# crabml/crabml

Measured on NVIDIA H100. Metric: decode_tokens_per_s, higher is better.
Workload: dtype int8

## Files before the change

### crabml_b200/csrc/mega.cu

```cuda
#define MK_SYNC() __syncthreads()
#include "mega_phases.cuh"

struct MkNextNorm { const float* norm_w; int norm_n; };

template <bool SMP>
__global__ void __launch_bounds__(MK_THREADS, MK_CTAS_PER_SM) mega_kernel(const MkPhase* __restrict__ phases, int n_phases, const uint8_t* dyn,
                                                                         unsigned* bar, const uint16_t* exp_lut, unsigned long long* prof, bool test_stall, int wtop_off,
                                                                         unsigned* err_host) {
    extern __shared__ __align__(16) uint8_t smem[];
    __shared__ float s_red[MK_WARPS];
    __shared__ MkPhase s_phs[2];
    __shared__ MkNextNorm s_next;
    __shared__ int s_abort;
    __shared__ __align__(8) unsigned long long s_abar[AT_NBUF];
    unsigned apar = 0u;
    const unsigned abar0 = (unsigned)__cvta_generic_to_shared(&s_abar[0]);
    if (threadIdx.x == 0) { for (int i = 0; i < AT_NBUF; i++) mbar_init(abar0 + 8u * i, 1u); s_abort = 0; }
    asm volatile("fence.mbarrier_init.release.cluster;" ::: "memory");
    asm volatile("fence.proxy.async.shared::cta;" ::: "memory");
    __syncthreads();
    const CommDev nocomm = {};
    KSeg S0, S1;
    uint8_t* work = smem;
    float* s_w = (float*)(smem + wtop_off);
    int wstaged = -1;
    int xstaged = -1;
    unsigned gen = 0;
    if (threadIdx.x == MK_BAR_THREAD) gen = ld_acquire_u32(&bar[32]);
    {
        const int* src = (const int*)phases;
        int* dst = (int*)&s_phs[0];
        for (int i = threadIdx.x; i < (int)(sizeof(MkPhase) / 4); i += MK_THREADS) dst[i] = src[i];
    }
    const int n_loop = SMP ? n_phases - 1 : n_phases;
    for (int p = 0; p < n_loop; p++) {
        const bool stamp = prof && blockIdx.x == 0 && threadIdx.x == 0;
        if (stamp) { prof[p * MK_PROF_SLOTS] = globaltimer_ns(); prof[p * MK_PROF_SLOTS + 1] = 0; prof[p * MK_PROF_SLOTS + 4] = 0; prof[p * MK_PROF_SLOTS + 5] = 0; }
        __syncthreads();
        const MkPhase& s_ph = s_phs[p & 1];
        static_assert(sizeof(MkPhase) / 4 <= MK_THREADS, "descriptor does not fit one word per thread");
        const int nx = s_ph.next_matvec;
        const bool look = nx > p && nx < n_phases;
        int desc_w = 0, next_w = 0;
        if (p + 1 < n_phases && threadIdx.x < sizeof(MkPhase) / 4) desc_w = ((const int*)(phases + p + 1))[threadIdx.x];
        if (look && threadIdx.x < 3) {
            const MkPhase* ph = phases + nx;
            next_w = threadIdx.x < 2 ? ((const int*)&ph->norm_w)[threadIdx.x] : ph->x && ph->norm_w && ph->norm_ahead ? ph->n : 0;
        }
        switch (s_ph.type) {
        case MK_NORMQ: phase_normq(s_ph, s_red); break;
        case MK_MATVEC: {
            unsigned long long* st1 = stamp ? prof + p * MK_PROF_SLOTS + 1 : nullptr;
            switch (s_ph.wtype) {
            case CC_Q2_K: phase_matvec_generic<TQ2_K>(s_ph, work, s_w, wstaged == p, xstaged == p, exp_lut, st1, S0, S1); break;
            case CC_Q3_K: phase_matvec_generic<TQ3_K>(s_ph, work, s_w, wstaged == p, xstaged == p, exp_lut, st1, S0, S1); break;
            case CC_Q4_K: phase_matvec_generic<TQ45_K<false>>(s_ph, work, s_w, wstaged == p, xstaged == p, exp_lut, st1, S0, S1); break;
            case CC_Q5_K: phase_matvec_generic<TQ45_K<true>>(s_ph, work, s_w, wstaged == p, xstaged == p, exp_lut, st1, S0, S1); break;
            case CC_Q6_K: phase_matvec_generic<TQ6_K>(s_ph, work, s_w, wstaged == p, xstaged == p, exp_lut, st1, S0, S1); break;
            default: phase_matvec_generic<TQ8_K>(s_ph, work, s_w, wstaged == p, xstaged == p, exp_lut, st1, S0, S1); break;
            }
            break;
        }
        case MK_ATTN:
            if (s_ph.at.kv_f16) phase_attn<true>(s_ph, (float*)work, s_red, dyn, exp_lut, abar0, apar, AT_CH); else phase_attn<false>(s_ph, (float*)work, s_red, dyn, exp_lut, abar0, apar, AT_CH);
            break;
        case MK_ROWS: phase_rows(s_ph, dyn); break;
        case MK_ARGMAX: phase_argmax(s_ph, dyn, s_red); break;
        }
        if (stamp) prof[p * MK_PROF_SLOTS + 2] = globaltimer_ns();
        if (p + 1 < n_phases && threadIdx.x < sizeof(MkPhase) / 4) ((int*)&s_phs[(p + 1) & 1])[threadIdx.x] = desc_w;
        if (look && threadIdx.x < 3) ((int*)&s_next)[threadIdx.x] = next_w;
        const bool more = p + 1 < n_phases;
        if (test_stall && p == 2 && blockIdx.x == gridDim.x - 1) { if (threadIdx.x == 0) s_abort = 1; break; }
        if (more) grid_barrier_arrive(bar, gridDim.x, gen);
        if (look && s_next.norm_n > 0) {
            const unsigned sw = (unsigned)__cvta_generic_to_shared(s_w);
            const float* nw = s_next.norm_w;
            for (int i = threadIdx.x; i < (s_next.norm_n >> 2); i += MK_THREADS)
                asm volatile("cp.async.cg.shared.global [%0], [%1], 16;" ::"r"(sw + i * 16), "l"(nw + i * 4) : "memory");
            asm volatile("cp.async.commit_group;" ::: "memory");
            wstaged = nx;
        }
        if (stamp) prof[p * MK_PROF_SLOTS + 3] = globaltimer_ns();
        if (more) {
            grid_barrier_wait(bar, gridDim.x, gen, nocomm, 0u, &s_abort, err_host);
            gen++;
            if (s_abort) break;
            const MkPhase& nph = s_phs[(p + 1) & 1];
            if (nph.type == MK_MATVEC && nph.x) {
                const unsigned sx = (unsigned)__cvta_generic_to_shared(work + mk_generic_sx_offset(nph.mv.k));
                const float* xg = nph.x;
                for (int i = threadIdx.x; i < (nph.mv.k >> 2); i += MK_THREADS)
                    asm volatile("cp.async.cg.shared.global [%0], [%1], 16;" ::"r"(sx + i * 16), "l"(xg + i * 4) : "memory");
                asm volatile("cp.async.commit_group;" ::: "memory");
                xstaged = p + 1;
            }
        }
    }
    asm volatile("cp.async.wait_all;" ::: "memory");
    if constexpr (SMP) {
        __syncthreads();
        if (!s_abort) phase_sample(s_phs[(n_phases - 1) & 1], dyn, work, exp_lut);
    }
    if (prof && blockIdx.x == 0 && threadIdx.x == 0) prof[n_phases * MK_PROF_SLOTS] = globaltimer_ns();
}

size_t cc_mega_smem_for_phase(const MkPhase& ph) {
    if (ph.type == MK_MATVEC) return (size_t)(((TKBase::smem_bytes(ph.mv.k) + 15) & ~15) + 256) + (size_t)ph.mv.k * 4;
    if (ph.type == MK_ATTN) return (size_t)(3 * ph.at.hd + ((ph.at.max_len + 8 + 3) & ~3) + AT_NBUF * AT_CH * ph.at.hd) * 4 + 64;
    if (ph.type == MK_SAMPLE) return SMP_SMEM_BYTES;
    return 1024;
}

extern "C" CC_API int cc_test_mega_barrier_floor(cc_device* dev, int n, float* us_per_phase) {
    if (!dev || n < 2 || !us_per_phase) return CC_ERR_ARG;
    std::vector<MkPhase> tab((size_t)n);
    for (auto& p : tab) { memset(&p, 0, sizeof(p)); p.type = 99; p.next_matvec = -1; }
// ... 49 lines not shown
```

### crabml_b200/csrc/mega_phases.cuh

```cuda
#pragma once
#include <stdlib.h>
#include <string.h>

#include "common.cuh"
#include "dequant.cuh"
#include "quantize_dev.cuh"
#include "vecdot.cuh"
#include "sample_dev.cuh"

#ifndef MK_SYNC
#error "define MK_SYNC() before including mega_phases.cuh"
#endif

#define MK_THREADS 512
#define MK_WARPS 16
#define MK_CTAS_PER_SM 1
#define MK_SEG 4
#define MK_XSTAGE_ROWS 512

__device__ __forceinline__ unsigned ld_acquire_u32(const unsigned* p) {
    unsigned v;
    asm volatile("ld.acquire.gpu.global.u32 %0, [%1];" : "=r"(v) : "l"(p) : "memory");
    return v;
}
// ... 203 lines not shown
    auto emit = [&](int i, float v) {
        int mat;
        const int r = locate(i, mat);
        if (pair) {
            if ((i & 1) == 0) { first = v; return; }
            flush_pending();
            if (lane == 0) { pend_a = first; pend_b = v; pend_row = r; pend_lut = exp_lut[f2h_bits(-first)]; }
        } else if (A.epilogue == 1) {
            flush_pending();
            if (lane == 0) { pend_a = v; pend_row = r; pend_res = ldcg_f(A.residual + r); }
        } else if (lane == 0) {
            float* o = mat == 0 ? M.out[0] : mat == 1 ? M.out[1] : M.out[2];
            o[r] = v;
        }
    };
    if constexpr (T::kSegmented) {
        const int NSEG = ((k >> 8) + 15) >> 4;
        const int U = n_vrows * NSEG;
#if MK_GENERIC_NOINLINE
        KSeg S0, S1;
#endif
        int x0[4] = {0, 0, 0, 0}, x1[4] = {0, 0, 0, 0};
        int l_i = 0, l_seg = 0;
        auto load = [&](KSeg& S, int (&x)[4], bool valid) {
            if (valid) { int mat; const int r = locate(l_i, mat); T::seg_load(S, x, planes(mat), r, k, l_seg, lane); }
            if (++l_seg == NSEG) { l_seg = 0; l_i++; }
        };
        load(S0, x0, U > 0);
        load(S1, x1, U > 1);
        float acc = 0.0f;
        int c_i = 0, c_seg = 0;
        auto finish = [&]() { if (++c_seg < NSEG) return; c_seg = 0; const float v = warp_sum(acc); acc = 0.0f; emit(c_i++, v); };
        for (int u = 0; u < U; u += 2) {
            acc = T::seg_dot(S0, x0, k, c_seg, smem, lane, acc);
            finish();
            load(S0, x0, u + 2 < U);
            if (u + 1 >= U) break;
            acc = T::seg_dot(S1, x1, k, c_seg, smem, lane, acc);
            finish();
            load(S1, x1, u + 3 < U);
        }
    } else {
        for (int i = 0; i < n_vrows; i++) {
            int mat;
            const int r = locate(i, mat);
            emit(i, warp_sum(T::row_dot(planes(mat), r, k, smem, lane)));
        }
    }
    flush_pending();
}

#define AT_CH 64
#define AT_NBUF 3
template <bool KV_F16>
static __device__ void phase_attn(const MkPhase& ph, float* sm, float* s_red, const uint8_t* dyn, const uint16_t* exp_lut, unsigned abar0, unsigned& apar, const int at_ch) {
    const AttnArgs& a = ph.at;
    const int n_heads = a.n_heads, n_kv = a.n_kv, hd = a.hd, rope_dim = a.rope_dim;
    const int64_t seq_stride = a.seq_stride;
    const int64_t* dynv = (const int64_t*)(dyn + ph.dyn_off);
    const float* rope_tab = (const float*)(dyn + ph.rope_off);
    const int kv_len = (int)dynv[1], L = kv_len + 1;
    const int lane = threadIdx.x & 31, warp = threadIdx.x >> 5;
    float* s_q = sm; float* s_k = sm + hd; float* s_v = sm + 2 * hd; float* s_p = sm + 3 * hd;
    uint8_t* s_buf = (uint8_t*)(sm + 3 * hd + ((a.max_len + 8 + 3) & ~3));
    const unsigned s_buf_smem = (unsigned)__cvta_generic_to_shared(s_buf);
    constexpr int ELT = KV_F16 ? 2 : 4;
    const unsigned buf_bytes = (unsigned)(at_ch * hd * ELT);
    const int pairs = rope_dim >> 1;
    const int hd4 = hd >> 2;
    const int NC = (kv_len + at_ch - 1) / at_ch;
    auto issue_job = [&](int g, int j) {
        const int c = j < NC ? j : j - NC;
        const int p0 = c * at_ch, cnt = min(at_ch, kv_len - p0);
        const uint8_t* src = (const uint8_t*)(j < NC ? a.kcache : a.vcache) + ((int64_t)g * seq_stride + (int64_t)p0 * hd) * ELT;
        const unsigned bytes = (unsigned)(cnt * hd * ELT), bar = abar0 + 8u * (unsigned)(j % AT_NBUF), dst = s_buf_smem + (unsigned)(j % AT_NBUF) * buf_bytes;
        asm volatile("mbarrier.arrive.expect_tx.shared::cta.b64 _, [%0], %1;" ::"r"(bar), "r"(bytes) : "memory");
        asm volatile("cp.async.bulk.shared::cluster.global.mbarrier::complete_tx::bytes [%0], [%1], %2, [%3];" ::"r"(dst), "l"(src), "r"(bytes), "r"(bar) : "memory");
    };
    auto wait_job = [&](int j) {
        const int bsel = j % AT_NBUF;
        mbar_wait(abar0 + 8u * (unsigned)bsel, (apar >> bsel) & 1u);
        apar ^= 1u << bsel;
    };
    auto ld_kv = [&](const uint8_t* buf, int idx) -> float { return KV_F16 ? __half2float(((const __half*)buf)[idx]) : ((const float*)buf)[idx]; };
    for (int h = blockIdx.x; h < n_heads; h += gridDim.x) {
        const int g = KV_F16 ? h / (n_heads / n_kv) : h % n_kv;
        if (threadIdx.x == 0) for (int j = 0; j < min(AT_NBUF, 2 * NC); j++) issue_job(g, j);
        for (int i = threadIdx.x; i < hd; i += MK_THREADS) {
            float qv, kvv;
            if (i < rope_dim) {
                const int j = i >> 1;
                const float c = rope_tab[j], s = rope_tab[pairs + j];
                const float q0 = ldcg_f(a.q + h * hd + 2 * j), q1 = ldcg_f(a.q + h * hd + 2 * j + 1);
                const float k0 = ldcg_f(a.k + g * hd + 2 * j), k1 = ldcg_f(a.k + g * hd + 2 * j + 1);
                qv = (i & 1) ? q0 * s + q1 * c : q0 * c - q1 * s;
                kvv = (i & 1) ? k0 * s + k1 * c : k0 * c - k1 * s;
            } else {
                qv = ldcg_f(a.q + h * hd + i);
                kvv = ldcg_f(a.k + g * hd + i);
            }
            s_q[i] = qv * a.scale;
            s_k[i] = kvv;
            s_v[i] = ldcg_f(a.v + g * hd + i);
        }
        MK_SYNC();
        const bool owner = KV_F16 ? (h % (n_heads / n_kv) == 0) : (h < n_kv);
        if (owner) {
            for (int i = threadIdx.x; i < hd; i += MK_THREADS) {
                const int64_t off = (int64_t)g * seq_stride + (int64_t)kv_len * hd + i;
                if (KV_F16) { ((__half*)a.kcache)[off] = __float2half_rn(s_k[i]); ((__half*)a.vcache)[off] = __float2half_rn(s_v[i]); }
                else { ((float*)a.kcache)[off] = s_k[i]; ((float*)a.vcache)[off] = s_v[i]; }
            }
        }
        for (int j = 0; j < NC; j++) {
            const int p0 = j * at_ch, cnt = min(at_ch, kv_len - p0);
            const uint8_t* kb = s_buf + (size_t)(j % AT_NBUF) * buf_bytes;
            wait_job(j);
            for (int s = warp; s < cnt; s += MK_WARPS) {
                float acc = 0.0f;
                for (int i = lane; i < hd; i += 32) acc += (KV_F16 ? __half2float(__float2half_rn(s_q[i])) : s_q[i]) * ld_kv(kb, s * hd + i);
                acc = warp_sum(acc);
                if (lane == 0) s_p[p0 + s] = acc;
            }
            MK_SYNC();
            if (threadIdx.x == 0 && j + AT_NBUF < 2 * NC) issue_job(g, j + AT_NBUF);
        }
        if (warp == 0) {
            float acc = 0.0f;
            for (int i = lane; i < hd; i += 32) {
                if (KV_F16) acc += __half2float(__float2half_rn(s_q[i])) * __half2float(__float2half_rn(s_k[i]));
                else acc += s_q[i] * s_k[i];
            }
            acc = warp_sum(acc);
            if (lane == 0) s_p[kv_len] = acc;
        }
        MK_SYNC();
        float m = -INFINITY;
        for (int s = threadIdx.x; s < L; s += MK_THREADS) m = fmaxf(m, s_p[s]);
        m = warp_max(m);
        if (lane == 0) s_red[warp] = m;
        MK_SYNC();
        m = s_red[0];
#pragma unroll
        for (int w = 1; w < MK_WARPS; w++) m = fmaxf(m, s_red[w]);
        MK_SYNC();
        float sum = 0.0f;
        for (int s = threadIdx.x; s < L; s += MK_THREADS) {
            float e = h2f_bits(exp_lut[f2h_bits(s_p[s] - m)]);
            s_p[s] = e;
            sum += e;
        }
        sum = warp_sum(sum);
        if (lane == 0) s_red[warp] = sum;
        MK_SYNC();
        sum = 0.0f;
#pragma unroll
        for (int w = 0; w < MK_WARPS; w++) sum += s_red[w];
        for (int s = threadIdx.x; s < L; s += MK_THREADS) s_p[s] = s_p[s] / sum;
        MK_SYNC();
        float accf = 0.0f;
        __half acch = __float2half_rn(0.0f);
        const int d = threadIdx.x;
        for (int j = NC; j < 2 * NC; j++) {
            const int p0 = (j - NC) * at_ch, cnt = min(at_ch, kv_len - p0);
            const uint8_t* vb = s_buf + (size_t)(j % AT_NBUF) * buf_bytes;
            wait_job(j);
            if (d < hd) {
                for (int s = 0; s < cnt; s++) {
                    if (KV_F16) acch = __hadd(acch, __hmul(((const __half*)vb)[s * hd + d], __float2half_rn(s_p[p0 + s])));
                    else accf += s_p[p0 + s] * ((const float*)vb)[s * hd + d];
                }
            }
            MK_SYNC();
            if (threadIdx.x == 0 && j + AT_NBUF < 2 * NC) issue_job(g, j + AT_NBUF);
        }
        float* s_o = s_k;
        MK_SYNC();
        if (d < hd) {
            float o;
            if (KV_F16) { acch = __hadd(acch, __hmul(__float2half_rn(s_v[d]), __float2half_rn(s_p[kv_len]))); o = __half2float(acch); }
            else { accf += s_p[kv_len] * s_v[d]; o = accf; }
            a.out[h * hd + d] = o;
            s_o[d] = o;
        }
        MK_SYNC();
        if (a.act_scratch) {
            ActQ8_0 act = ph.act;
            for (int b = warp; b < (hd >> 5); b += MK_WARPS) {
                float v = s_o[b * 32 + lane];
                float amax = warp_max(fabsf(v));
                float dd = amax / 127.0f;
                int qq = __float2int_rz(v / dd);
                const int gb = h * (hd >> 5) + b;
                act.qs[gb * 32 + lane] = (int8_t)qq;
                int ss = warp_sum_i(qq);
                if (lane == 0) { act.d[gb] = __half2float(__float2half_rn(dd)); act.isum[gb] = ss; }
            }
        }
        MK_SYNC();
    }
}

static __device__ void phase_rows(const MkPhase& ph, const uint8_t* dyn) {
    const int64_t* rows = ph.rows_dev ? (const int64_t*)ph.rows_dev : (const int64_t*)(dyn + ph.dyn_off);
    const int64_t total = (int64_t)ph.n_rows * ph.cols;
    for (int64_t i = (int64_t)blockIdx.x * MK_THREADS + threadIdx.x; i < total; i += (int64_t)gridDim.x * MK_THREADS) {
        const int64_t r = i / ph.cols, c = i - r * ph.cols;
        const int64_t e = rows[r] * ph.cols + c;
        float v;
        if (ph.src_dtype == CC_F32) v = __ldcg((const float*)ph.planes.p[0] + e);
        else if (ph.src_dtype == CC_F16) v = __half2float(((const __half*)ph.planes.p[0])[e]);
        else v = dequant_elem(ph.src_dtype, ph.planes, e);
        if (ph.dst_dtype == CC_F32) ((float*)ph.dst)[i] = v; else ((__half*)ph.dst)[i] = __float2half_rn(v);
    }
}

static __device__ void phase_argmax(const MkPhase& ph, const uint8_t* dyn, float* s_red) {
    if (blockIdx.x != 0) return;
// ... 70 lines not shown
```

### crabml_b200/csrc/mega_ring.cu

```cuda
#define MK_SYNC() asm volatile("bar.sync 1, 512;" ::: "memory")
#define MK_GENERIC_NOINLINE 1
#include "mega_phases.cuh"

#define MR_PRODUCER_WARPS 4
#define MR_THREADS (MK_THREADS + 32 * MR_PRODUCER_WARPS)
#define MR_MAX_SLOTS 112
#define MR_Q8_SLOTS 24
#define MR_DESC_WORDS ((int)(sizeof(MkPhase) / 4))
#define MR_DESC_PER_LANE ((MR_DESC_WORDS + 31) / 32)

struct MrRing {
    int ring_off;
    int slot_bytes;
    int nslots;
    int at_ch;
};

__device__ __forceinline__ void mr_expect_tx(unsigned bar, unsigned bytes) { asm volatile("mbarrier.arrive.expect_tx.shared::cta.b64 _, [%0], %1;" ::"r"(bar), "r"(bytes) : "memory"); }
__device__ __forceinline__ void mr_bulk_g2s(unsigned dst, const void* src, unsigned bytes, unsigned bar, unsigned long long pol) {
    asm volatile("cp.async.bulk.shared::cluster.global.mbarrier::complete_tx::bytes.L2::cache_hint [%0], [%1], %2, [%3], %4;" ::"r"(dst), "l"(src), "r"(bytes), "r"(bar), "l"(pol) : "memory");
}
__device__ __forceinline__ void mr_stage_f32(float* dst, const float* src, int n) {
    const unsigned s = (unsigned)__cvta_generic_to_shared(dst);
    for (int i = threadIdx.x; i < (n >> 2); i += MK_THREADS) asm volatile("cp.async.cg.shared.global [%0], [%1], 16;" ::"r"(s + i * 16), "l"(src + i * 4) : "memory");
    asm volatile("cp.async.commit_group;" ::: "memory");
}
__host__ __device__ __forceinline__ int mr_nbp(int k) { const int GR = ((k >> 5) + 31) >> 5; return (GR + MK_SEG - 1) / MK_SEG * MK_SEG * 32; }
__host__ __device__ __forceinline__ int mr_x_off(int k) { return mr_nbp(k) * 40 + 256 + 2048; }
__device__ __forceinline__ bool mr_try_wait(unsigned bar, unsigned parity) {
    unsigned ok;
    asm volatile("{\n.reg .pred p;\nmbarrier.try_wait.parity.shared::cta.b64 p, [%1], %2;\nselp.u32 %0, 1, 0, p;\n}\n" : "=r"(ok) : "r"(bar), "r"(parity) : "memory");
    return ok != 0;
}
__device__ __forceinline__ void mr_release(unsigned done_addr, unsigned v, float dep) { asm volatile("st.release.cta.shared::cta.u32 [%0], %1;" ::"r"(done_addr), "r"(v), "f"(dep) : "memory"); }
__device__ __forceinline__ unsigned mr_ld_acquire_shared(unsigned addr) {
    unsigned v;
    asm volatile("ld.acquire.cta.shared::cta.u32 %0, [%1];" : "=r"(v) : "r"(addr) : "memory");
    return v;
}

struct MrGeo {
    int nb, GR, NSEG, V, E, n_units, first, stride, last_half_off, m_cat;
    bool pair;
};
__device__ __forceinline__ MrGeo mr_geo(const StreamArgs& A) {
    MrGeo g;
    g.nb = A.k >> 5; g.GR = (g.nb + 31) >> 5; g.NSEG = (g.GR + MK_SEG - 1) / MK_SEG;
    g.pair = A.epilogue == 2;
    const StreamMats& M = A.mats;
    g.m_cat = g.pair ? M.m[0] : M.m[0] + (M.n > 1 ? M.m[1] : 0) + (M.n > 2 ? M.m[2] : 0);
    if (A.epilogue == 3) {
        const int rpc = (((g.m_cat + (int)gridDim.x - 1) / (int)gridDim.x) + 3) & ~3;
        g.first = (int)blockIdx.x * rpc; g.stride = 1;
        g.n_units = min(rpc, max(0, g.m_cat - g.first));
    } else {
        g.first = (int)blockIdx.x; g.stride = (int)gridDim.x;
        g.n_units = g.first < g.m_cat ? (g.m_cat - g.first + g.stride - 1) / g.stride : 0;
    }
    g.V = g.pair ? 2 : 1;
    g.E = g.V * g.NSEG;
    g.last_half_off = 16 * (g.nb - 32 * (g.GR - 1));
    return g;
}
__device__ __forceinline__ int mr_locate(const StreamMats& M, const MrGeo& g, int rc, int v, int& mat) {
    mat = 0;
    int r = rc;
    if (g.pair) { mat = v; return r; }
    if (M.n > 1 && r >= M.m[0]) { r -= M.m[0]; mat = 1; if (M.n > 2 && r >= M.m[1]) { r -= M.m[1]; mat = 2; } }
    return r;
}

__device__ void mr_producer(const MkPhase* __restrict__ phases, int n_phases, const MrRing R, unsigned full0, unsigned done0, unsigned ring0,
                            MkPhase* s_pd, volatile unsigned* s_seq, volatile int* s_abort, int* s_prod_done, unsigned long long* prof_tail) {
    const int lane = threadIdx.x & 31;
    const int pt = (int)threadIdx.x - MK_THREADS;
    unsigned long long p_trips = 0, p_cyc = 0, p_iss = 0;
    unsigned long long pol;
    asm volatile("createpolicy.fractional.L2::evict_first.b64 %0, 1.0;" : "=l"(pol));
    for (int i = lane; i < MR_DESC_WORDS; i += 32) ((int*)&s_pd[0])[i] = ((const int*)phases)[i];
    __syncwarp();
    unsigned ent = 0;
// ... 79 lines not shown
__device__ __forceinline__ int mr_act_word(int i) {
    const int b = i >> 3, w = i & 7;
    return (b >> 5) * 256 + (w >> 2) * 128 + (b & 31) * 4 + (w & 3);
}
__device__ __forceinline__ int mr_act_int4(int i) {
    const int b = i >> 1;
    return (b >> 5) * 64 + (i & 1) * 32 + (b & 31);
}

template <int TYPE>
__device__ __forceinline__ void mr_dot2(const uint8_t* spA, const uint8_t* spB, int seg, int nb, int GR, int last_half_off, int lane,
                                        const int4* aq_l, const float* ad_l, const int* as_l, float& partA, float& partB) {
    constexpr int GB = TYPE == CC_Q8_0 ? 1024 : 512;
    const uint8_t* qA = spA + lane * 16;
    const uint8_t* qB = spB + lane * 16;
    const uint16_t* dA = (const uint16_t*)(spA + MK_SEG * GB) + lane;
    const uint16_t* dB = (const uint16_t*)(spB + MK_SEG * GB) + lane;
    const int4* aq = aq_l + seg * (MK_SEG * 64);
    const float* ad = ad_l + seg * (MK_SEG * 32);
    const int4 z4 = make_int4(0, 0, 0, 0);
    float accA = 0.0f, accB = 0.0f;
#pragma unroll
    for (int g = 0; g < MK_SEG; g++) {
        const int gi = seg * MK_SEG + g;
        const bool on = gi * 32 + lane < nb;
        const int4 alo = aq[g * 64], ahi = aq[g * 64 + 32];
        const float adv = ad[g * 32];
        if constexpr (TYPE == CC_Q8_0) {
            const int hoff = gi == GR - 1 ? last_half_off : 512;
            int4 a0 = z4, a1 = z4, b0 = z4, b1 = z4; uint16_t sA = 0, sB = 0;
            if (on) { a0 = *(const int4*)(qA + g * GB); a1 = *(const int4*)(qA + g * GB + hoff); sA = dA[g * 32];
                      b0 = *(const int4*)(qB + g * GB); b1 = *(const int4*)(qB + g * GB + hoff); sB = dB[g * 32]; }
            const int sumA = mk_dp16(a0, alo) + mk_dp16(a1, ahi);
            const int sumB = mk_dp16(b0, alo) + mk_dp16(b1, ahi);
            accA += (float)sumA * h2f_bits(sA) * adv;
            accB += (float)sumB * h2f_bits(sB) * adv;
        } else {
            int4 wA = z4, wB = z4; uint16_t sA = 0, sB = 0;
            if (on) { wA = *(const int4*)(qA + g * GB); sA = dA[g * 32]; wB = *(const int4*)(qB + g * GB); sB = dB[g * 32]; }
            const int asv = as_l[(seg * MK_SEG + g) * 32];
            const int4 loA = make_int4(wA.x & 0x0F0F0F0F, wA.y & 0x0F0F0F0F, wA.z & 0x0F0F0F0F, wA.w & 0x0F0F0F0F);
            const int4 hiA = make_int4((wA.x >> 4) & 0x0F0F0F0F, (wA.y >> 4) & 0x0F0F0F0F, (wA.z >> 4) & 0x0F0F0F0F, (wA.w >> 4) & 0x0F0F0F0F);
            const int4 loB = make_int4(wB.x & 0x0F0F0F0F, wB.y & 0x0F0F0F0F, wB.z & 0x0F0F0F0F, wB.w & 0x0F0F0F0F);
            const int4 hiB = make_int4((wB.x >> 4) & 0x0F0F0F0F, (wB.y >> 4) & 0x0F0F0F0F, (wB.z >> 4) & 0x0F0F0F0F, (wB.w >> 4) & 0x0F0F0F0F);
            const int sumA = mk_dp16(loA, alo) + mk_dp16(hiA, ahi) - 8 * asv;
            const int sumB = mk_dp16(loB, alo) + mk_dp16(hiB, ahi) - 8 * asv;
            accA += (float)sumA * h2f_bits(sA) * adv;
            accB += (float)sumB * h2f_bits(sB) * adv;
        }
    }
    partA = accA; partB = accB;
}

template <int TYPE>
__device__ void phase_matvec_ring(const MkPhase& ph, uint8_t* smem, float* s_wn, const float*& wst, bool x_staged, const uint16_t* exp_lut, MrCons& RC,
                                  const CommDev& comm, unsigned xseq, unsigned long long* stamp1) {
    const StreamArgs& A = ph.mv;
    const int k = A.k;
    const MrGeo g = mr_geo(A);
    const int nb = g.nb, GR = g.GR, NSEG = g.NSEG;
    const bool pair = g.pair;
    const int nbp = NSEG * MK_SEG * 32;
    int8_t* s_q = (int8_t*)smem;
    float* s_d = (float*)(smem + (size_t)nbp * 32);
    int* s_s = (int*)(smem + (size_t)nbp * 32 + (size_t)nbp * 4);
    float* s_red = (float*)(smem + (size_t)nbp * 40);
    float* s_part = (float*)(smem + (size_t)nbp * 40 + 256);
    const int lane = threadIdx.x & 31, warp = threadIdx.x >> 5;
    const StreamMats& M = A.mats;
    if (threadIdx.x == 0) *RC.s_unit = 0;
    if (ph.x) {
        const int n4 = k >> 2;
        const int npass = nbp >> 6;
        const float4 z4 = make_float4(0, 0, 0, 0);
        const float4* s_w4 = (const float4*)s_wn;
        const float4* s_x4 = (const float4*)(smem + mr_x_off(k));
        const float* xbase = ph.red_n ? comm.data[comm.rank] + (size_t)(xseq & 1u) * CC_COMM_MAX_RANKS * CC_COMM_MAX_ELEMS : ph.x;
        auto load_x = [&](int i) -> float4 {
            if (i >= n4) return z4;
            if (!ph.red_n) return s_x4[i];
            float4 a4 = __ldcg((const float4*)xbase + i);
            for (int p = 1; p < comm.world; p++) {
                const float4 t4 = __ldcg((const float4*)(xbase + (size_t)p * CC_COMM_MAX_ELEMS) + i);
                a4.x += t4.x; a4.y += t4.y; a4.z += t4.z; a4.w += t4.w;
            }
            if (ph.red_res) { const float4 r4 = __ldcg((const float4*)ph.red_res + i); a4.x += r4.x; a4.y += r4.y; a4.z += r4.z; a4.w += r4.w; }
            return a4;
        };
        if (ph.norm_w && ph.norm_w != wst) { mr_stage_f32(s_wn, ph.norm_w, k); wst = ph.norm_w; }
        if (!ph.red_n && !x_staged) mr_stage_f32((float*)s_x4, ph.x, k);
        asm volatile("cp.async.wait_group 1;" ::: "memory");
        if (stamp1) stamp1[7] = globaltimer_ns();
        asm volatile("cp.async.wait_group 0;" ::: "memory");
        if (stamp1) stamp1[3] = globaltimer_ns();
        float rms = 1.0f;
        const bool in_regs = ph.red_n && npass <= 4;
        float4 xr[4];
#pragma unroll
        for (int j = 0; j < 4; j++) xr[j] = z4;
        if (in_regs) {
#pragma unroll
            for (int j = 0; j < 4; j++) if (j < npass) xr[j] = load_x(j * MK_THREADS + (int)threadIdx.x);
        }
        if (ph.norm_w) {
            float ss = 0.0f;
            if (in_regs) {
#pragma unroll
                for (int j = 0; j < 4; j++) if (j * MK_THREADS + (int)threadIdx.x < n4) ss += cc_sq4(xr[j]);
            } else {
// ... 21 lines not shown
            const int q0 = live ? __float2int_rz(v.x / d) : 0, q1 = live ? __float2int_rz(v.y / d) : 0;
            const int q2 = live ? __float2int_rz(v.z / d) : 0, q3 = live ? __float2int_rz(v.w / d) : 0;
            s_q32[mr_act_word(i)] = (q0 & 255) | ((q1 & 255) << 8) | ((q2 & 255) << 16) | (q3 << 24);
            if constexpr (TYPE == CC_Q4_0) {
                int sq = q0 + q1 + q2 + q3;
#pragma unroll
                for (int o = 4; o > 0; o >>= 1) sq += __shfl_xor_sync(0xffffffffu, sq, o);
                if (sub == 0) s_s[i >> 3] = sq;
            }
            if (sub == 0) s_d[i >> 3] = live ? __half2float(__float2half_rn(d)) : 0.0f;
        };
        auto load_w = [&](int i) -> float4 { return ph.norm_w && i < n4 ? s_w4[i] : z4; };
        if (in_regs) {
#pragma unroll
            for (int j = 0; j < 4; j++) if (j < npass) quant_chunk(j * MK_THREADS + (int)threadIdx.x, xr[j], load_w(j * MK_THREADS + (int)threadIdx.x));
        } else if (!ph.red_n) {
            for (int j = 0; j < npass; j++) { const int i = j * MK_THREADS + (int)threadIdx.x; quant_chunk(i, load_x(i), load_w(i)); }
        } else {
            for (int j0 = 0; j0 < npass; j0 += 4) {
                float4 v[4];
#pragma unroll
                for (int j = 0; j < 4; j++) v[j] = j0 + j < npass ? load_x((j0 + j) * MK_THREADS + (int)threadIdx.x) : z4;
#pragma unroll
                for (int j = 0; j < 4; j++) if (j0 + j < npass) quant_chunk((j0 + j) * MK_THREADS + (int)threadIdx.x, v[j], load_w((j0 + j) * MK_THREADS + (int)threadIdx.x));
            }
        }
    } else {
        const uint8_t* act = (const uint8_t*)A.act;
        const int4* gq = (const int4*)act;
        int4* sq4 = (int4*)s_q;
        const float* gd = (const float*)(act + ((k + 15) & ~15));
        const int* gs = (const int*)(act + ((k + 15) & ~15) + ((nb * 4 + 15) & ~15));
        if (nbp <= MK_THREADS) {
            const int i0 = threadIdx.x, i1 = threadIdx.x + MK_THREADS;
            const int4 z4 = make_int4(0, 0, 0, 0);
            const int4 qa = i0 < nb * 2 ? __ldcg(gq + i0) : z4, qb = i1 < nb * 2 ? __ldcg(gq + i1) : z4;
            const float dv = i0 < nb ? __ldcg(gd + i0) : 0.0f;
            int sv = 0;
            if constexpr (TYPE == CC_Q4_0) sv = i0 < nb ? __ldcg(gs + i0) : 0;
            if (i0 < nbp * 2) sq4[mr_act_int4(i0)] = qa;
            if (i1 < nbp * 2) sq4[mr_act_int4(i1)] = qb;
            if (i0 < nbp) { s_d[i0] = dv; if constexpr (TYPE == CC_Q4_0) s_s[i0] = sv; }
        } else {
            for (int i = threadIdx.x; i < nbp * 2; i += MK_THREADS) sq4[mr_act_int4(i)] = i < nb * 2 ? __ldcg(gq + i) : make_int4(0, 0, 0, 0);
            for (int i = threadIdx.x; i < nbp; i += MK_THREADS) {
                s_d[i] = i < nb ? __ldcg(gd + i) : 0.0f;
                if constexpr (TYPE == CC_Q4_0) s_s[i] = i < nb ? __ldcg(gs + i) : 0;
            }
        }
    }
    MK_SYNC();
    if (stamp1) *stamp1 = globaltimer_ns();
    if (ph.x && ph.norm_w) { wst = ph.next_norm_w; if (wst) mr_stage_f32(s_wn, wst, ph.next_norm_n); }
    const int4* aq_l = (const int4*)s_q + lane;
    const float* ad_l = s_d + lane;
    const int* as_l = s_s + lane;
    float pend_a[2] = {0.0f, 0.0f}, pend_b[2] = {0.0f, 0.0f}, pend_res[2] = {0.0f, 0.0f};
    unsigned short pend_lut[2] = {0, 0};
    int pend_row[2] = {-1, -1};
    auto flush_pending = [&]() {
#pragma unroll
        for (int t = 0; t < 2; t++) {
            if (lane == 0 && pend_row[t] >= 0) {
                if (pair) M.out[0][pend_row[t]] = (pend_a[t] / (1.0f + h2f_bits(pend_lut[t]))) * pend_b[t];
                else M.out[0][pend_row[t]] = pend_a[t] + pend_res[t];
            }
            pend_row[t] = -1;
        }
    };
    long long c_wait = 0, c_all = 0; int c_n = 0;
    if (stamp1) c_all = clock64();
    const unsigned NS = (unsigned)RC.nslots;
    const int npairs = g.n_units >> 1, twoE = 2 * g.E;
    const bool pairs = g.n_units > 1;
    for (;;) {
        int P = 0;
        if (lane == 0) P = atomicAdd(RC.s_unit, 1);
        P = __shfl_sync(0xffffffffu, P, 0);
        const bool two = pairs && P < npairs;
        if (pairs ? (!two && !(P == npairs && (g.n_units & 1))) : P >= g.n_units) break;
        const int u0 = !pairs ? P : two ? 2 * P : g.n_units - 1;
        const unsigned step = two ? 2u : 1u;
        unsigned eA = RC.ent_base + (unsigned)(!pairs ? P * g.E : two ? P * twoE : npairs * twoE);
        unsigned slotA = eA % NS, parA = (eA / NS) & 1u;
        float first[2] = {0.0f, 0.0f};
        for (int v = 0; v < g.V; v++) {
            float accA = 0.0f, accB = 0.0f;
            for (int sg = 0; sg < NSEG; sg++) {
                unsigned slotB = slotA + 1u, parB = parA;
                if (slotB == NS) { slotB = 0; parB ^= 1u; }
                long long t0 = 0;
                if (stamp1) t0 = clock64();
                mr_wait_full(RC, slotA, eA, parA);
                if (two) mr_wait_full(RC, slotB, eA + 1u, parB);
                if (stamp1) { c_wait += clock64() - t0; c_n += two ? 2 : 1; }
                const uint8_t* spA = RC.ring + (size_t)slotA * RC.slot_bytes;
                const uint8_t* spB = two ? RC.ring + (size_t)slotB * RC.slot_bytes : spA;
                float partA, partB;
                mr_dot2<TYPE>(spA, spB, sg, nb, GR, g.last_half_off, lane, aq_l, ad_l, as_l, partA, partB);
                accA += partA; accB += partB;
                __syncwarp();
                if (lane == 0) { mr_release(RC.done0 + 4u * slotA, eA + 1u, partA); if (two) mr_release(RC.done0 + 4u * slotB, eA + 2u, partB); }
                eA += step; slotA += step;
                if (slotA >= NS) { slotA -= NS; parA ^= 1u; }
            }
            const float rA = warp_sum(accA), rB = warp_sum(accB);
            if (pair && v == 0) { first[0] = rA; first[1] = rB; continue; }
            if (pair || A.epilogue == 1) flush_pending();
#pragma unroll
            for (int t = 0; t < 2; t++) {
                if (t == 1 && !two) break;
                const float r = t ? rB : rA;
                const int u = u0 + t, rc = g.first + u * g.stride;
                if (lane != 0) continue;
                if (pair) { pend_a[t] = first[t]; pend_b[t] = r; pend_row[t] = rc; pend_lut[t] = exp_lut[f2h_bits(-first[t])]; }
                else if (A.epilogue == 1) { pend_a[t] = r; pend_row[t] = rc; pend_res[t] = ldcg_f(A.residual + rc); }
                else if (A.epilogue == 3) s_part[u] = r;
                else {
                    int mat;
                    const int rr = mr_locate(M, g, rc, 0, mat);
                    float* o = mat == 0 ? M.out[0] : mat == 1 ? M.out[1] : M.out[2];
                    o[rr] = r;
                }
            }
        }
    }
    flush_pending();
    if (stamp1) { stamp1[5] = (unsigned long long)c_wait; stamp1[6] = ((unsigned long long)(clock64() - c_all) << 20) | (unsigned long long)c_n; }
    RC.ent_base += (unsigned)(g.n_units * g.E);
    if (A.epilogue == 3) {
        MK_SYNC();
        if (warp < comm.world) {
            const size_t off = ((size_t)((xseq + 1u) & 1u) * CC_COMM_MAX_RANKS + comm.rank) * CC_COMM_MAX_ELEMS + g.first;
            for (int c4 = lane * 4; c4 < g.n_units; c4 += 128) *(float4*)(comm.data[warp] + off + c4) = *(const float4*)(s_part + c4);
        }
    }
}

template <bool GEN, bool SMP>
__global__ void __launch_bounds__(MR_THREADS, 1) mega_ring_kernel(const MkPhase* __restrict__ phases, int n_phases, const uint8_t* dyn, unsigned* bar,
                                                                  const uint16_t* exp_lut, unsigned long long* prof, bool test_stall, int wtop_off, unsigned* err_host,
                                                                  const CommDev comm, const MrRing R) {
    extern __shared__ __align__(128) uint8_t smem[];
    __shared__ float s_red[MK_WARPS];
    __shared__ MkPhase s_phs[2];
    __shared__ MkPhase s_pd[MR_PRODUCER_WARPS][2];
    __shared__ int s_abort;
    __shared__ int s_prod_done;
    __shared__ int s_ring_dead;
    __shared__ int s_unit;
    __shared__ __align__(8) unsigned long long s_abar[AT_NBUF];
    __shared__ __align__(8) unsigned long long s_full[MR_MAX_SLOTS];
    __shared__ unsigned s_done[MR_MAX_SLOTS];
    __shared__ unsigned s_seq[MR_MAX_SLOTS];
    unsigned apar = 0u;
    const unsigned abar0 = (unsigned)__cvta_generic_to_shared(&s_abar[0]);
    const unsigned full0 = (unsigned)__cvta_generic_to_shared(&s_full[0]);
    const unsigned done0 = (unsigned)__cvta_generic_to_shared(&s_done[0]);
    if (threadIdx.x == 0) {
        for (int i = 0; i < AT_NBUF; i++) mbar_init(abar0 + 8u * i, 1u);
        for (int i = 0; i < R.nslots; i++) { mbar_init(full0 + 8u * i, 1u); s_done[i] = 0u; s_seq[i] = 0u; }
        s_abort = 0; s_prod_done = 0; s_ring_dead = 0;
    }
    asm volatile("fence.mbarrier_init.release.cluster;" ::: "memory");
    asm volatile("fence.proxy.async.shared::cta;" ::: "memory");
    __syncthreads();
    if (threadIdx.x >= MK_THREADS) {
        mr_producer(phases, n_phases, R, full0, done0, (unsigned)__cvta_generic_to_shared(smem + R.ring_off), s_pd[(threadIdx.x - MK_THREADS) >> 5], s_seq, &s_abort, &s_prod_done,
                    prof ? prof + (size_t)n_phases * MK_PROF_SLOTS : nullptr);
        return;
    }
    MrCons RC;
    RC.full0 = full0; RC.done0 = done0; RC.ring = smem + R.ring_off; RC.slot_bytes = R.slot_bytes; RC.nslots = R.nslots; RC.ent_base = 0u;
    RC.s_unit = &s_unit; RC.s_seq = s_seq; RC.s_dead = &s_ring_dead; RC.err_dev = &bar[MK_BAR_ERR]; RC.err_host = err_host;
    uint8_t* work = smem;
    float* s_wn = (float*)(smem + wtop_off);
    const float* wst = nullptr;
    int xstaged = -1;
    unsigned gen = 0;
    if (threadIdx.x == MK_BAR_THREAD) gen = ld_acquire_u32(&bar[32]);
    unsigned xseq = comm.world > 0 ? *comm.seq : 0u;
    for (int i = threadIdx.x; i < MR_DESC_WORDS; i += MK_THREADS) ((int*)&s_phs[0])[i] = ((const int*)phases)[i];
    const int n_loop = SMP ? n_phases - 1 : n_phases;
    for (int p = 0; p < n_loop; p++) {
        const bool stamp = prof && blockIdx.x == 0 && threadIdx.x == 0;
        if (stamp) { prof[p * MK_PROF_SLOTS] = globaltimer_ns(); prof[p * MK_PROF_SLOTS + 1] = 0; prof[p * MK_PROF_SLOTS + 4] = 0; prof[p * MK_PROF_SLOTS + 5] = 0; prof[p * MK_PROF_SLOTS + 8] = 0; }
        MK_SYNC();
        const MkPhase& s_ph = s_phs[p & 1];
        if (p == 0 && !(s_ph.type == MK_MATVEC && s_ph.x && s_ph.norm_w)) { wst = s_ph.next_norm_w; if (wst) mr_stage_f32(s_wn, wst, s_ph.next_norm_n); }
        static_assert(sizeof(MkPhase) / 4 <= MK_THREADS, "descriptor does not fit one word per thread");
        int desc_w = 0;
        if (p + 1 < n_phases && threadIdx.x < sizeof(MkPhase) / 4) desc_w = ((const int*)(phases + p + 1))[threadIdx.x];
        unsigned long long* st1 = stamp ? prof + p * MK_PROF_SLOTS + 1 : nullptr;
        switch (s_ph.type) {
        case MK_NORMQ: phase_normq(s_ph, s_red); break;
        case MK_MATVEC:
            if (GEN && s_ph.act_type == CC_Q8_K) {
                switch (s_ph.wtype) {
                case CC_Q2_K: phase_matvec_generic<TQ2_K>(s_ph, work, s_wn, s_ph.norm_w == wst, false, exp_lut, st1); break;
                case CC_Q3_K: phase_matvec_generic<TQ3_K>(s_ph, work, s_wn, s_ph.norm_w == wst, false, exp_lut, st1); break;
                case CC_Q4_K: phase_matvec_generic<TQ45_K<false>>(s_ph, work, s_wn, s_ph.norm_w == wst, false, exp_lut, st1); break;
                case CC_Q5_K: phase_matvec_generic<TQ45_K<true>>(s_ph, work, s_wn, s_ph.norm_w == wst, false, exp_lut, st1); break;
                case CC_Q6_K: phase_matvec_generic<TQ6_K>(s_ph, work, s_wn, s_ph.norm_w == wst, false, exp_lut, st1); break;
                default: phase_matvec_generic<TQ8_K>(s_ph, work, s_wn, s_ph.norm_w == wst, false, exp_lut, st1); break;
                }
                if (s_ph.x && s_ph.norm_w) { wst = s_ph.next_norm_w; if (wst) mr_stage_f32(s_wn, wst, s_ph.next_norm_n); }
                break;
            }
            if (s_ph.wtype == CC_Q8_0) phase_matvec_ring<CC_Q8_0>(s_ph, work, s_wn, wst, xstaged == p, exp_lut, RC, comm, xseq, st1);
            else phase_matvec_ring<CC_Q4_0>(s_ph, work, s_wn, wst, xstaged == p, exp_lut, RC, comm, xseq, st1);
            break;
        case MK_ATTN:
            if (s_ph.at.kv_f16) phase_attn<true>(s_ph, (float*)work, s_red, dyn, exp_lut, abar0, apar, R.at_ch);
            else phase_attn<false>(s_ph, (float*)work, s_red, dyn, exp_lut, abar0, apar, R.at_ch);
            break;
        case MK_ROWS: phase_rows(s_ph, dyn); break;
        case MK_REDUCE: phase_reduce(s_ph, comm, xseq, false); break;
        case MK_GATHER: phase_reduce(s_ph, comm, xseq, true); break;
        case MK_ARGMAX: phase_argmax(s_ph, dyn, s_red); break;
        }
        if (stamp) prof[p * MK_PROF_SLOTS + 2] = globaltimer_ns();
        if (p + 1 < n_phases && threadIdx.x < sizeof(MkPhase) / 4) ((int*)&s_phs[(p + 1) & 1])[threadIdx.x] = desc_w;
        const bool more = p + 1 < n_phases;
        const bool xg = s_ph.xgpu != 0;
        if (test_stall && p == 2 && blockIdx.x == gridDim.x - 1) { if (threadIdx.x == 0) s_abort = 1; break; }
        if (more) grid_barrier_arrive(bar, gridDim.x, gen);
        if (stamp) prof[p * MK_PROF_SLOTS + 3] = globaltimer_ns();
        if (more) {
            grid_barrier_wait(bar, gridDim.x, gen, comm, xg ? xseq + 1u : 0u, &s_abort, err_host);
            gen++; if (xg) xseq++;
            if (s_abort) break;
            const MkPhase& nph = s_phs[(p + 1) & 1];
            if (nph.type == MK_MATVEC && nph.act_type != CC_Q8_K && nph.x && !nph.red_n) { mr_stage_f32((float*)(work + mr_x_off(nph.mv.k)), nph.x, nph.mv.k); xstaged = p + 1; }
        }
    }
    asm volatile("cp.async.wait_all;" ::: "memory");
    if constexpr (SMP) {
        MK_SYNC();
        if (!s_abort) phase_sample(s_phs[(n_phases - 1) & 1], dyn, work, exp_lut);
    }
    if (comm.world > 0 && blockIdx.x == 0 && threadIdx.x == 0) *comm.seq = xseq;
    if (prof && blockIdx.x == 0 && threadIdx.x == 0) prof[n_phases * MK_PROF_SLOTS] = globaltimer_ns();
    MK_SYNC();
    if (s_abort && threadIdx.x == 0) {
        while (*(volatile int*)&s_prod_done < MR_PRODUCER_WARPS) {}
        for (unsigned sl = 0; sl < (unsigned)R.nslots; sl++) {
            const unsigned q = *(volatile unsigned*)&s_seq[sl];
            if (q) mbar_wait(full0 + 8u * sl, ((q - 1u) / (unsigned)R.nslots) & 1u);
        }
    }
}

bool cc_mega_ring_phase_ok(const MkPhase& ph) {
    if (ph.type != MK_MATVEC || ph.act_type == CC_Q8_K) return true;
    if (ph.wtype != CC_Q8_0 && ph.wtype != CC_Q4_0) return false;
    if (ph.mv.k % 32) return false;
    for (int t = 0; t < ph.mv.mats.n; t++)
        if (((uintptr_t)ph.mv.mats.qs[t] | (uintptr_t)ph.mv.mats.d[t]) & 15u) return false;
    return true;
}
int cc_mega_ring_at_ch(const MkPhase& ph) {
    return ph.at.kv_f16 ? 64 : 32;
}
size_t cc_mega_ring_smem_for_phase(const MkPhase& ph) {
    if (ph.type == MK_MATVEC && ph.act_type == CC_Q8_K) return cc_mega_smem_for_phase(ph);
    if (ph.type == MK_MATVEC) return (size_t)mr_x_off(ph.mv.k) + (ph.x && !ph.red_n ? (size_t)ph.mv.k * 4 : 0);
    if (ph.type == MK_ATTN) return (size_t)(3 * ph.at.hd + ((ph.at.max_len + 8 + 3) & ~3)) * 4 + (size_t)AT_NBUF * cc_mega_ring_at_ch(ph) * ph.at.hd * (ph.at.kv_f16 ? 2 : 4) + 64;
    if (ph.type == MK_SAMPLE) return SMP_SMEM_BYTES;
    return 1024;
}
#define MR_MIN_SLOTS 12
static size_t mr_ring_off(const MegaLaunch& L) { return ((((L.smem + 15) & ~(size_t)15) + L.wstage) + 127) & ~(size_t)127; }
static auto mr_kernel(const MegaLaunch& L) {
    return L.generic ? (L.sample ? mega_ring_kernel<true, true> : mega_ring_kernel<true, false>) : (L.sample ? mega_ring_kernel<false, true> : mega_ring_kernel<false, false>);
}
int cc_mega_ring_slots(const MegaLaunch& L) {
    cudaFuncAttributes fa;
    if (cudaFuncGetAttributes(&fa, mr_kernel(L)) != cudaSuccess) { cudaGetLastError(); return 0; }
    const size_t cap = 227 * 1024 - fa.sharedSizeBytes, off = mr_ring_off(L);
    if (L.slot_bytes <= 0 || off >= cap) return 0;
    const int fit = (int)std::min((cap - off) / (size_t)L.slot_bytes, (size_t)MR_MAX_SLOTS);
    if (fit < MR_MIN_SLOTS) return 0;
    return L.slot_bytes >= 4352 ? std::min(fit, MR_Q8_SLOTS) : fit;
}

int cc_launch_mega_ring(cc_device* dev, const MkPhase* phases_dev, int n_phases, const uint8_t* dyn_dev, unsigned* bar_dev, const MegaLaunch& L,
                        unsigned long long* prof, const CommDev* comm) {
    auto kern = mr_kernel(L);
    const size_t wtop = (L.smem + 15) & ~(size_t)15;
// ... 16 lines not shown
```

Before: 280.0.

## Prefetch attention KV chunks during preceding ring matvec phase

Moves the attention staging buffers to grow downward from the top of the work area. In the ring kernel, the matvec phase before an attention phase now issues the first bulk async copies of this block's KV cache chunks early, when smem space above the matvec area allows. The goal is to hide KV load latency behind the matvec and the grid barrier. In exchange it adds cross-phase mbarrier state (at_pf), a drain wait at kernel exit, and a non-inlined attention function, with some risk of smem overlap or parity errors.

After: 285.1 (median of 6 runs). 1.8% higher.

```diff
diff --git a/crabml_b200/csrc/mega.cu b/crabml_b200/csrc/mega.cu
--- a/crabml_b200/csrc/mega.cu
+++ b/crabml_b200/csrc/mega.cu
@@ -62,7 +62,8 @@
             break;
         }
         case MK_ATTN:
-            if (s_ph.at.kv_f16) phase_attn<true>(s_ph, (float*)work, s_red, dyn, exp_lut, abar0, apar, AT_CH); else phase_attn<false>(s_ph, (float*)work, s_red, dyn, exp_lut, abar0, apar, AT_CH);
+            if (s_ph.at.kv_f16) phase_attn<true>(s_ph, (float*)work, s_red, dyn, exp_lut, abar0, apar, AT_CH, wtop_off, 0);
+            else phase_attn<false>(s_ph, (float*)work, s_red, dyn, exp_lut, abar0, apar, AT_CH, wtop_off, 0);
             break;
         case MK_ROWS: phase_rows(s_ph, dyn); break;
         case MK_ARGMAX: phase_argmax(s_ph, dyn, s_red); break;
diff --git a/crabml_b200/csrc/mega_phases.cuh b/crabml_b200/csrc/mega_phases.cuh
--- a/crabml_b200/csrc/mega_phases.cuh
+++ b/crabml_b200/csrc/mega_phases.cuh
@@ -279,31 +279,43 @@
 
 #define AT_CH 64
 #define AT_NBUF 3
+__device__ __forceinline__ unsigned at_buf_smem(unsigned buf_top_smem, unsigned buf_bytes, int b) { return buf_top_smem - (unsigned)(b + 1) * buf_bytes; }
+__device__ __forceinline__ void at_issue_job(const AttnArgs& a, int g, int j, int kv_len, int at_ch, int elt, unsigned abar0, unsigned buf_top_smem) {
+    const int NC = (kv_len + at_ch - 1) / at_ch;
+    const int c = j < NC ? j : j - NC;
+    const int p0 = c * at_ch, cnt = min(at_ch, kv_len - p0);
+    const uint8_t* src = (const uint8_t*)(j < NC ? a.kcache : a.vcache) + ((int64_t)g * a.seq_stride + (int64_t)p0 * a.hd) * elt;
+    const unsigned bytes = (unsigned)(cnt * a.hd * elt), bar = abar0 + 8u * (unsigned)(j % AT_NBUF);
+    const unsigned dst = at_buf_smem(buf_top_smem, (unsigned)(at_ch * a.hd * elt), j % AT_NBUF);
+    asm volatile("mbarrier.arrive.expect_tx.shared::cta.b64 _, [%0], %1;" ::"r"(bar), "r"(bytes) : "memory");
+    asm volatile("cp.async.bulk.shared::cluster.global.mbarrier::complete_tx::bytes [%0], [%1], %2, [%3];" ::"r"(dst), "l"(src), "r"(bytes), "r"(bar) : "memory");
+}
+__device__ __forceinline__ int at_kv_head(const AttnArgs& a, int h) { return a.kv_f16 ? h / (a.n_heads / a.n_kv) : h % a.n_kv; }
+#ifndef MK_ATTN_NOINLINE
+#define MK_ATTN_NOINLINE 0
+#endif
+#if MK_ATTN_NOINLINE
+#define MK_ATTN_ATTR __noinline__
+#else
+#define MK_ATTN_ATTR
+#endif
 template <bool KV_F16>
-static __device__ void phase_attn(const MkPhase& ph, float* sm, float* s_red, const uint8_t* dyn, const uint16_t* exp_lut, unsigned abar0, unsigned& apar, const int at_ch) {
+static __device__ MK_ATTN_ATTR void phase_attn(const MkPhase& ph, float* sm, float* s_red, const uint8_t* dyn, const uint16_t* exp_lut, unsigned abar0, unsigned& apar, const int at_ch,
+                                  int buf_top, int npf) {
     const AttnArgs& a = ph.at;
     const int n_heads = a.n_heads, n_kv = a.n_kv, hd = a.hd, rope_dim = a.rope_dim;
-    const int64_t seq_stride = a.seq_stride;
     const int64_t* dynv = (const int64_t*)(dyn + ph.dyn_off);
     const float* rope_tab = (const float*)(dyn + ph.rope_off);
     const int kv_len = (int)dynv[1], L = kv_len + 1;
     const int lane = threadIdx.x & 31, warp = threadIdx.x >> 5;
     float* s_q = sm; float* s_k = sm + hd; float* s_v = sm + 2 * hd; float* s_p = sm + 3 * hd;
-    uint8_t* s_buf = (uint8_t*)(sm + 3 * hd + ((a.max_len + 8 + 3) & ~3));
-    const unsigned s_buf_smem = (unsigned)__cvta_generic_to_shared(s_buf);
+    const unsigned buf_top_smem = (unsigned)__cvta_generic_to_shared(sm) + (unsigned)buf_top;
     constexpr int ELT = KV_F16 ? 2 : 4;
     const unsigned buf_bytes = (unsigned)(at_ch * hd * ELT);
+    const uint8_t* s_buf0 = (const uint8_t*)sm + buf_top;
     const int pairs = rope_dim >> 1;
-    const int hd4 = hd >> 2;
     const int NC = (kv_len + at_ch - 1) / at_ch;
-    auto issue_job = [&](int g, int j) {
-        const int c = j < NC ? j : j - NC;
-        const int p0 = c * at_ch, cnt = min(at_ch, kv_len - p0);
-        const uint8_t* src = (const uint8_t*)(j < NC ? a.kcache : a.vcache) + ((int64_t)g * seq_stride + (int64_t)p0 * hd) * ELT;
-        const unsigned bytes = (unsigned)(cnt * hd * ELT), bar = abar0 + 8u * (unsigned)(j % AT_NBUF), dst = s_buf_smem + (unsigned)(j % AT_NBUF) * buf_bytes;
-        asm volatile("mbarrier.arrive.expect_tx.shared::cta.b64 _, [%0], %1;" ::"r"(bar), "r"(bytes) : "memory");
-        asm volatile("cp.async.bulk.shared::cluster.global.mbarrier::complete_tx::bytes [%0], [%1], %2, [%3];" ::"r"(dst), "l"(src), "r"(bytes), "r"(bar) : "memory");
-    };
+    auto issue_job = [&](int g, int j) { at_issue_job(a, g, j, kv_len, at_ch, ELT, abar0, buf_top_smem); };
     auto wait_job = [&](int j) {
         const int bsel = j % AT_NBUF;
         mbar_wait(abar0 + 8u * (unsigned)bsel, (apar >> bsel) & 1u);
@@ -311,8 +323,8 @@
     };
     auto ld_kv = [&](const uint8_t* buf, int idx) -> float { return KV_F16 ? __half2float(((const __half*)buf)[idx]) : ((const float*)buf)[idx]; };
     for (int h = blockIdx.x; h < n_heads; h += gridDim.x) {
-        const int g = KV_F16 ? h / (n_heads / n_kv) : h % n_kv;
-        if (threadIdx.x == 0) for (int j = 0; j < min(AT_NBUF, 2 * NC); j++) issue_job(g, j);
+        const int g = at_kv_head(a, h);
+        if (threadIdx.x == 0) for (int j = h == (int)blockIdx.x ? npf : 0; j < min(AT_NBUF, 2 * NC); j++) issue_job(g, j);
         for (int i = threadIdx.x; i < hd; i += MK_THREADS) {
             float qv, kvv;
             if (i < rope_dim) {
@@ -334,14 +346,14 @@
         const bool owner = KV_F16 ? (h % (n_heads / n_kv) == 0) : (h < n_kv);
         if (owner) {
             for (int i = threadIdx.x; i < hd; i += MK_THREADS) {
-                const int64_t off = (int64_t)g * seq_stride + (int64_t)kv_len * hd + i;
+                const int64_t off = (int64_t)g * a.seq_stride + (int64_t)kv_len * hd + i;
                 if (KV_F16) { ((__half*)a.kcache)[off] = __float2half_rn(s_k[i]); ((__half*)a.vcache)[off] = __float2half_rn(s_v[i]); }
                 else { ((float*)a.kcache)[off] = s_k[i]; ((float*)a.vcache)[off] = s_v[i]; }
             }
         }
         for (int j = 0; j < NC; j++) {
             const int p0 = j * at_ch, cnt = min(at_ch, kv_len - p0);
-            const uint8_t* kb = s_buf + (size_t)(j % AT_NBUF) * buf_bytes;
+            const uint8_t* kb = s_buf0 - (size_t)(j % AT_NBUF + 1) * buf_bytes;
             wait_job(j);
             for (int s = warp; s < cnt; s += MK_WARPS) {
                 float acc = 0.0f;
@@ -390,7 +402,7 @@
         const int d = threadIdx.x;
         for (int j = NC; j < 2 * NC; j++) {
             const int p0 = (j - NC) * at_ch, cnt = min(at_ch, kv_len - p0);
-            const uint8_t* vb = s_buf + (size_t)(j % AT_NBUF) * buf_bytes;
+            const uint8_t* vb = s_buf0 - (size_t)(j % AT_NBUF + 1) * buf_bytes;
             wait_job(j);
             if (d < hd) {
                 for (int s = 0; s < cnt; s++) {
diff --git a/crabml_b200/csrc/mega_ring.cu b/crabml_b200/csrc/mega_ring.cu
--- a/crabml_b200/csrc/mega_ring.cu
+++ b/crabml_b200/csrc/mega_ring.cu
@@ -1,5 +1,6 @@
 #define MK_SYNC() asm volatile("bar.sync 1, 512;" ::: "memory")
 #define MK_GENERIC_NOINLINE 1
+#define MK_ATTN_NOINLINE 1
 #include "mega_phases.cuh"
 
 #define MR_PRODUCER_WARPS 4
@@ -27,6 +28,7 @@
 }
 __host__ __device__ __forceinline__ int mr_nbp(int k) { const int GR = ((k >> 5) + 31) >> 5; return (GR + MK_SEG - 1) / MK_SEG * MK_SEG * 32; }
 __host__ __device__ __forceinline__ int mr_x_off(int k) { return mr_nbp(k) * 40 + 256 + 2048; }
+__host__ __device__ __forceinline__ int mr_area(const MkPhase& ph) { return mr_x_off(ph.mv.k) + (ph.x && !ph.red_n ? ph.mv.k * 4 : 0); }
 __device__ __forceinline__ bool mr_try_wait(unsigned bar, unsigned parity) {
     unsigned ok;
     asm volatile("{\n.reg .pred p;\nmbarrier.try_wait.parity.shared::cta.b64 p, [%1], %2;\nselp.u32 %0, 1, 0, p;\n}\n" : "=r"(ok) : "r"(bar), "r"(parity) : "memory");
@@ -212,9 +214,26 @@
     partA = accA; partB = accB;
 }
 
+static __device__ __noinline__ int mr_attn_prefetch(const MkPhase& ph, const MkPhase* nph, const uint8_t* dyn, uint8_t* work, int wtop, unsigned abar0, int at_ch) {
+    if (nph->type != MK_ATTN) return 0;
+    const AttnArgs& a = nph->at;
+    const int h = (int)blockIdx.x;
+    if (h >= a.n_heads) return 0;
+    const int kv_len = (int)((const int64_t*)(dyn + nph->dyn_off))[1];
+    const int elt = a.kv_f16 ? 2 : 4, bb = at_ch * a.hd * elt, jobs = 2 * ((kv_len + at_ch - 1) / at_ch), lo = mr_area(ph);
+    int n = 0;
+    while (n < AT_NBUF && n < jobs && wtop - (n + 1) * bb >= lo) n++;
+    if (!n) return 0;
+    asm volatile("fence.proxy.async;" ::: "memory");
+    const unsigned top = (unsigned)__cvta_generic_to_shared(work) + (unsigned)wtop;
+    for (int j = 0; j < n; j++) at_issue_job(a, at_kv_head(a, h), j, kv_len, at_ch, elt, abar0, top);
+    return n;
+}
+
 template <int TYPE>
 __device__ void phase_matvec_ring(const MkPhase& ph, uint8_t* smem, float* s_wn, const float*& wst, bool x_staged, const uint16_t* exp_lut, MrCons& RC,
-                                  const CommDev& comm, unsigned xseq, unsigned long long* stamp1) {
+                                  const CommDev& comm, unsigned xseq, unsigned long long* stamp1, const MkPhase* nph, const uint8_t* dyn, int wtop,
+                                  unsigned abar0, int at_ch, int& at_pf) {
     const StreamArgs& A = ph.mv;
     const int k = A.k;
     const MrGeo g = mr_geo(A);
@@ -342,6 +361,7 @@
     MK_SYNC();
     if (stamp1) *stamp1 = globaltimer_ns();
     if (ph.x && ph.norm_w) { wst = ph.next_norm_w; if (wst) mr_stage_f32(s_wn, wst, ph.next_norm_n); }
+    if (threadIdx.x == 0 && nph) at_pf = mr_attn_prefetch(ph, nph, dyn, smem, wtop, abar0, at_ch);
     const int4* aq_l = (const int4*)s_q + lane;
     const float* ad_l = s_d + lane;
     const int* as_l = s_s + lane;
@@ -444,6 +464,7 @@
     __shared__ unsigned s_done[MR_MAX_SLOTS];
     __shared__ unsigned s_seq[MR_MAX_SLOTS];
     unsigned apar = 0u;
+    int at_pf = 0;
     const unsigned abar0 = (unsigned)__cvta_generic_to_shared(&s_abar[0]);
     const unsigned full0 = (unsigned)__cvta_generic_to_shared(&s_full[0]);
     const unsigned done0 = (unsigned)__cvta_generic_to_shared(&s_done[0]);
@@ -497,12 +518,16 @@
                 if (s_ph.x && s_ph.norm_w) { wst = s_ph.next_norm_w; if (wst) mr_stage_f32(s_wn, wst, s_ph.next_norm_n); }
                 break;
             }
-            if (s_ph.wtype == CC_Q8_0) phase_matvec_ring<CC_Q8_0>(s_ph, work, s_wn, wst, xstaged == p, exp_lut, RC, comm, xseq, st1);
-            else phase_matvec_ring<CC_Q4_0>(s_ph, work, s_wn, wst, xstaged == p, exp_lut, RC, comm, xseq, st1);
+            {
+                const MkPhase* nph = p + 1 < n_phases ? phases + p + 1 : nullptr;
+                if (s_ph.wtype == CC_Q8_0) phase_matvec_ring<CC_Q8_0>(s_ph, work, s_wn, wst, xstaged == p, exp_lut, RC, comm, xseq, st1, nph, dyn, wtop_off, abar0, R.at_ch, at_pf);
+                else phase_matvec_ring<CC_Q4_0>(s_ph, work, s_wn, wst, xstaged == p, exp_lut, RC, comm, xseq, st1, nph, dyn, wtop_off, abar0, R.at_ch, at_pf);
+            }
             break;
         case MK_ATTN:
-            if (s_ph.at.kv_f16) phase_attn<true>(s_ph, (float*)work, s_red, dyn, exp_lut, abar0, apar, R.at_ch);
-            else phase_attn<false>(s_ph, (float*)work, s_red, dyn, exp_lut, abar0, apar, R.at_ch);
+            if (s_ph.at.kv_f16) phase_attn<true>(s_ph, (float*)work, s_red, dyn, exp_lut, abar0, apar, R.at_ch, wtop_off, at_pf);
+            else phase_attn<false>(s_ph, (float*)work, s_red, dyn, exp_lut, abar0, apar, R.at_ch, wtop_off, at_pf);
+            at_pf = 0;
             break;
         case MK_ROWS: phase_rows(s_ph, dyn); break;
         case MK_REDUCE: phase_reduce(s_ph, comm, xseq, false); break;
@@ -525,6 +550,7 @@
         }
     }
     asm volatile("cp.async.wait_all;" ::: "memory");
+    for (int j = 0; j < at_pf; j++) mbar_wait(abar0 + 8u * j, (apar >> j) & 1u);
     if constexpr (SMP) {
         MK_SYNC();
         if (!s_abort) phase_sample(s_phs[(n_phases - 1) & 1], dyn, work, exp_lut);
```
